# brendan-duncan/unity_webgpu_pathtracer

Measured on AMD Instinct MI355X. Metric: Mrays/s at 1920x1080, 8 spp, higher is better.
Workload: dtype f32; 1 GPU; sponza: Sponza-class atrium (~250k tris, 24 textured Disney materials, 2 rect lights + sky), 1920x1080, 8 spp/pass, depth 4, progressive passes (CurrentSample = 8k); tris=250752, schedule=1, passes_in_flight=12, passes_per_launch_sequence=1

## Files before the change

### unity_webgpu_pathtracer_amd/csrc/pt_device.h

```cpp
#pragma once

#include <hip/hip_runtime.h>
#include <stdint.h>
#include "ptmi_layouts.h"
#include "ptmi_math.h"
#include "ptmi_plugin.h"

#define PT_DEV __device__ __forceinline__

struct v2 { float x, y; };
struct v3 { float x, y, z; };
struct v4 { float x, y, z, w; };

PT_DEV v3 mk3(float a) { return {a, a, a}; }
PT_DEV v3 mk3(float a, float b, float c) { return {a, b, c}; }
PT_DEV v3 operator+(v3 a, v3 b) { return {a.x + b.x, a.y + b.y, a.z + b.z}; }
PT_DEV v3 operator-(v3 a, v3 b) { return {a.x - b.x, a.y - b.y, a.z - b.z}; }
PT_DEV v3 operator-(v3 a) { return {-a.x, -a.y, -a.z}; }
PT_DEV v3 operator*(v3 a, v3 b) { return {a.x * b.x, a.y * b.y, a.z * b.z}; }
PT_DEV v3 operator*(v3 a, float s) { return {a.x * s, a.y * s, a.z * s}; }
PT_DEV v3 operator*(float s, v3 a) { return {s * a.x, s * a.y, s * a.z}; }
PT_DEV v3 operator/(v3 a, float s) { return {a.x / s, a.y / s, a.z / s}; }
PT_DEV v3 operator-(float s, v3 a) { return {s - a.x, s - a.y, s - a.z}; }
PT_DEV v4 operator+(v4 a, v4 b) { return {a.x + b.x, a.y + b.y, a.z + b.z, a.w + b.w}; }
// ... 1232 lines not shown
    v3 Li = light.emission * falloff;
    out.dir = lsDirection;
    out.valid = 1u;
    float pdf = 0.0f;
    v3 f = eval_brdf_onb(mat, -rayDir, lsDirection, onb_of_normal(hit.normal, hit.ffnormal, ffOnb), pdf, sh);
    float lightPdf = 1.0f;
    if (lsPdf > 0.0f) lightPdf = lsPdf;
    out.contribution = Li * f / lightPdf;
}

PT_DEV v4 mul44(const float* m, v4 v)
{
    v4 r;
    r.x = m[0] * v.x + m[4] * v.y + m[8] * v.z + m[12] * v.w;
    r.y = m[1] * v.x + m[5] * v.y + m[9] * v.z + m[13] * v.w;
    r.z = m[2] * v.x + m[6] * v.y + m[10] * v.z + m[14] * v.w;
    r.w = m[3] * v.x + m[7] * v.y + m[11] * v.z + m[15] * v.w;
    return r;
}

PT_DEV void concentric_sample_disk(float u1, float u2, float& dx, float& dy)
{
    float sx = 2.0f * u1 - 1.0f;
    float sy = 2.0f * u2 - 1.0f;
    if (sx == 0.0f && sy == 0.0f) { dx = 0.0f; dy = 0.0f; return; }
    float r, theta;
    if (sx >= -sy) {
        if (sx > sy) { r = sx; theta = sy > 0.0f ? sy / r : 8.0f + sy / r; }
        else { r = sy; theta = 2.0f - sx / r; }
    } else {
        if (sx <= sy) { r = -sx; theta = 4.0f - sy / r; }
        else { r = -sy; theta = 6.0f + sx / r; }
    }
    theta *= PT_PI / 4.0f;
    dx = r * pt_cos(theta);
    dy = r * pt_sin(theta);
}

PT_DEV void generate_camera_ray(const PTFrameParams& P, uint32_t pixelX, uint32_t pixelY, uint32_t& rng, v3& origin, v3& direction)
{
    float g0 = rnd(rng);
    float g1 = rnd(rng);
    float gr = pt_sqrt(-2.0f * pt_log(pt_max(1e-38f, g0)));
    float gtheta = 2.0f * PT_PI * g1;
    float gx = gr * pt_cos(gtheta), gy = gr * pt_sin(gtheta);
    float pcx = (float)pixelX + (0.5f + PT_AA_SIGMA * gx);
    float pcy = (float)pixelY + (0.5f + PT_AA_SIGMA * gy);

    v4 o4 = mul44(P.CamToWorld, v4{0.0f, 0.0f, 0.0f, 1.0f});
    origin = mk3(o4.x, o4.y, o4.z);
    float uvx = pcx / (float)P.OutputWidth * 2.0f - 1.0f;
    float uvy = pcy / (float)P.OutputHeight * 2.0f - 1.0f;
    v4 d4 = mul44(P.CamInvProj, v4{uvx, uvy, 0.0f, 1.0f});
    v4 w4 = mul44(P.CamToWorld, v4{d4.x, d4.y, d4.z, 0.0f});
    direction = normalize3(mk3(w4.x, w4.y, w4.z));
    if (P.Aperture > 0.0f && P.FocalLength > 0.0f) {
        float sampleLensU = rnd(rng);
        float sampleLensV = rnd(rng);
        float lensU, lensV;
        concentric_sample_disk(sampleLensU, sampleLensV, lensU, lensV);
        float lensRadius = P.Aperture * 0.5f;
        lensU *= lensRadius;
        lensV *= lensRadius;
        float ft = P.FocalLength;
        v3 focalPoint = origin + direction * ft;
        v4 l4 = mul44(P.CamToWorld, v4{lensU, lensV, 0.0f, 1.0f});
        origin = mk3(l4.x, l4.y, l4.z);
        direction = normalize3(focalPoint - origin);
    }
}

enum : uint32_t { PS_TRACE = 0u, PS_ENDING = 1u, PS_DONE = 2u };

struct PathRegs {
    v3 ro, rd;
    v3 radiance, throughput, color;
    float scatterPdf, maxRoughness;
    uint32_t rng, depth, state, sampleIdx;
    NeeRay env, light;
    v3 neeOrigin, pendThroughput;
    bool hasPending, green;
};

PT_DEV void path_start_sample(const PTFrameParams& P, uint32_t pixelX, uint32_t pixelY, PathRegs& r, Counters& cn)
{
    cn.paths++;
    r.radiance = mk3(0.0f);
    r.throughput = mk3(1.0f);
    r.depth = 0u;
    r.scatterPdf = 0.0f;
    r.maxRoughness = 0.0f;
    generate_camera_ray(P, pixelX, pixelY, r.rng, r.ro, r.rd);
    r.state = PS_TRACE;
}

PT_DEV void path_init(const PTFrameParams& P, uint32_t seedRoot, uint32_t currentSample, uint32_t pixelX, uint32_t pixelY, uint32_t pixelIndex,
                      PathRegs& r, Counters& cn)
{
    r.rng = pixelIndex * (currentSample + 1u) + seedRoot;
    r.sampleIdx = 0u;
    r.color = mk3(0.0f);
    r.env.valid = 0u; r.light.valid = 0u;
    r.env.dir = mk3(0.0f); r.light.dir = mk3(0.0f);
    r.env.contribution = mk3(0.0f); r.light.contribution = mk3(0.0f);
    r.neeOrigin = mk3(0.0f); r.pendThroughput = mk3(0.0f);
    r.hasPending = false; r.green = false;
    path_start_sample(P, pixelX, pixelY, r, cn);
}

struct NoNeeSink { PT_DEV void operator()(PathRegs&) const {} };
struct CameraSample {
    PT_DEV void operator()(const PTFrameParams& P, uint32_t pixelX, uint32_t pixelY, PathRegs& r, Counters& cn) const { path_start_sample(P, pixelX, pixelY, r, cn); }
};

PT_DEV void path_apply_pending(PathRegs& r, bool occEnv, bool occLight)
{
    if (r.hasPending) {
        v3 Ld = mk3(0.0f);
        if (r.env.valid == 1u && !occEnv) Ld = Ld + r.env.contribution;
        if (r.light.valid == 1u && !occLight) Ld = Ld + r.light.contribution;
        r.radiance = r.radiance + Ld * r.pendThroughput;
        if (r.green) r.radiance = mk3(0.0f, 1.0f, 0.0f);
        r.hasPending = false;
        r.green = false;
    }
}

template <bool STATS, class NeeSink = NoNeeSink>
PT_DEV void path_shade_hit(const DScene& S, const PTFrameParams& P, PathRegs& r, const HitRecord& rec, Counters& cn, NeeSink neeSink = NeeSink())
{
    {
        const uint32_t maxRayBounces = P.MaxRayBounces > 1u ? P.MaxRayBounces : 1u;
        SurfHit hit;
        hit.distance = PT_FAR_PLANE;
        hit.isLight = 0u;
        hit.triIndex = 0u;
        hit.materialIndex = 0;
        hit.position = mk3(0.0f); hit.normal = mk3(0.0f); hit.ffnormal = mk3(0.0f);
        hit.uv = {0.0f, 0.0f};
        if (rec.h.t < PT_FAR_PLANE) {
            if (S.hasTlas) fetch_hit_attributes_tlas(S, r.rd, rec, hit);
            else fetch_hit_attributes<STATS>(S, r.ro, r.rd, rec.h, hit, cn);
        }
        intersect_lights<STATS>(S, r.ro, r.rd, hit, cn);

        if (!(hit.distance < PT_FAR_PLANE)) {
            v4 sky = sample_sky_radiance(S, P, r.rd, r.depth);
            float misWeight = 1.0f;
            if (r.depth > 0u) misWeight = power_heuristic(r.scatterPdf, sky.w);
            if (misWeight > 0.0f) r.radiance = r.radiance + misWeight * mk3(sky.x, sky.y, sky.z) * r.throughput;
            r.state = PS_ENDING;
        } else if (S.hasLights && hit.isLight) {
            DLight light = load_light(S, (int)hit.triIndex);
            if (STATS) cn.lightFetches++;
            r.radiance = r.radiance + light.emission * r.throughput;
            r.state = PS_ENDING;
        } else {
            Material material = get_material<STATS>(S, hit.materialIndex, r.rd, hit, cn);
            r.maxRoughness = pt_max(r.maxRoughness, material.roughness);
            material.roughness = r.maxRoughness;
            r.radiance = r.radiance + material.emission * r.throughput;
            if (r.depth >= maxRayBounces) {
                r.state = PS_ENDING;
            } else {
                v3 scatterL;
                const float alphaRnd = rnd(r.rng);
                const bool skip = (material.alphaMode == (float)PT_ALPHA_MODE_MASK && material.opacity < material.alphaCutoff) ||
                                  (material.alphaMode == (float)PT_ALPHA_MODE_BLEND && alphaRnd > material.opacity);
                bool advance = true;
                if (skip) {
                    scatterL = r.rd;
                } else {
                    r.neeOrigin = nee_scatter_pos(hit);
                    BsdfShared sh;
                    tint_colors(material, material.eta, sh.F0, sh.Csheen, sh.Cspec0);
                    const Onb ffOnb = make_onb(hit.ffnormal);
                    nee_prepare_environment(S, P, r.rd, hit, material, r.rng, r.env, sh, ffOnb);
                    nee_prepare_light<STATS>(S, r.rd, hit, material, r.neeOrigin, r.rng, r.light, cn, sh, ffOnb);
                    r.pendThroughput = r.throughput;
                    r.hasPending = true;
                    neeSink(r);
                    float pdf;
                    v3 f = sample_brdf(material, -r.rd, ffOnb, scatterL, pdf, r.rng, sh);
                    r.scatterPdf = pdf;
                    if (pt_isnan(f.x) || pt_isnan(f.y) || pt_isnan(f.z)) {
                        r.green = true;
                        r.state = PS_ENDING;
                        advance = false;
                    } else if (pdf > 0.0f) {
                        r.throughput = r.throughput * (f / pdf);
                    } else {
                        r.state = PS_ENDING;
                        advance = false;
                    }
                    if (advance) r.depth++;
                }
                if (advance) {
                    r.rd = scatterL;
                    r.ro = hit.position + r.rd * PT_EPSILON;
                    if (P.UseRussianRoulette) {
                        float rrPcont = pt_min(pt_max(r.throughput.x, pt_max(r.throughput.y, r.throughput.z)) + 0.001f, 0.95f);
                        if (rnd(r.rng) >= rrPcont) r.state = PS_ENDING;
                        else r.throughput = r.throughput / rrPcont;
                    }
                }
            }
        }
    }
}

template <bool INLINE_RESOLVE, class Source = CameraSample>
PT_DEV void path_end_sample(const PTFrameParams& P, PathRegs& r, uint32_t pixelX, uint32_t pixelY, uint32_t pixelIndex,
                            const float4* __restrict__ accumulated, float4* __restrict__ output, Counters& cn, Source source = Source())
{
    if (r.state == PS_ENDING && !r.hasPending) {
        if (P.UseFireflyFilter) {
            float lum = luminance3(r.radiance);
            if (lum > P.MaxFireflyLuminance) r.radiance = r.radiance * (P.MaxFireflyLuminance / lum);
        }
        r.color = r.color + r.radiance;
        r.sampleIdx++;
        const uint32_t numSamples = P.SamplesPerPass > 1 ? (uint32_t)P.SamplesPerPass : 1u;
        if (r.sampleIdx < numSamples) {
            source(P, pixelX, pixelY, r, cn);
        } else if (!INLINE_RESOLVE) {
            r.state = PS_DONE;
        } else {
            const float fSamples = (float)numSamples;
            float4 o4;
            if (P.CurrentSample > 0u) {
                float4 a = accumulated[pixelIndex];
                cn.pixelsRead++;
                float cs = (float)P.CurrentSample;
                v3 acc = (r.color + mk3(a.x, a.y, a.z) * cs) / (cs + fSamples);
                o4 = make_float4(acc.x, acc.y, acc.z, 1.0f);
            } else {
                v3 acc = r.color / fSamples;
                o4 = make_float4(acc.x, acc.y, acc.z, 1.0f);
            }
            output[pixelIndex] = o4;
            cn.pixelsWritten++;
            r.state = PS_DONE;
        }
    }
}

template <bool STATS, bool INLINE_RESOLVE = true, class NeeSink = NoNeeSink, class Source = CameraSample>
PT_DEV void path_step(const DScene& S, const PTFrameParams& P, PathRegs& r, const HitRecord& rec, bool occEnv, bool occLight,
                      uint32_t pixelX, uint32_t pixelY, uint32_t pixelIndex,
                      const float4* __restrict__ accumulated, float4* __restrict__ output, Counters& cn, NeeSink neeSink = NeeSink(),
                      Source source = Source())
{
    path_apply_pending(r, occEnv, occLight);
    if (r.state == PS_TRACE) path_shade_hit<STATS, NeeSink>(S, P, r, rec, cn, neeSink);
    path_end_sample<INLINE_RESOLVE, Source>(P, r, pixelX, pixelY, pixelIndex, accumulated, output, cn, source);
}

PT_DEV uint32_t wave_sum_u32(uint32_t v)
{
#pragma unroll
    for (int off = 32; off > 0; off >>= 1) v += __shfl_xor(v, off, 64);
    return v;
}
PT_DEV uint32_t wave_max_u32(uint32_t v)
{
#pragma unroll
    for (int off = 32; off > 0; off >>= 1) { uint32_t o = __shfl_xor(v, off, 64); v = o > v ? o : v; }
    return v;
}
#define PT_NUM_COUNTERS 16
PT_DEV void counters_to_array(const Counters& cn, uint32_t* vals)
{
    vals[0] = cn.paths; vals[1] = cn.closestRays; vals[2] = cn.shadowRays; vals[3] = cn.nodeVisits; vals[4] = cn.triTests;
    vals[5] = cn.attrFetches; vals[6] = cn.materialFetches; vals[7] = cn.lightFetches; vals[8] = cn.texelFetches;
    vals[9] = cn.texDescFetches; vals[10] = cn.pixelsWritten; vals[11] = cn.pixelsRead; vals[12] = cn.maxStack; vals[13] = cn.overflows;
    vals[14] = cn.tlasNodeVisits; vals[15] = cn.instanceVisits;
}

template <bool STATS, class ST>
PT_DEV bool ray_step(const DScene& S, RayState& r, ST& st, Counters& cn)
{
    return cwbvh_iteration<STATS, false>(S, r, BlasOffsets{}, st, cn);
}

template <bool STATS>
PT_DEV bool ray_tri_one(const DScene& S, RayState& r, Counters& cn)
{
    const uint32_t triangleIndex = 31u - (uint32_t)__clz((int)r.tg.y);
    intersect_triangle<false>(S.tris, r.tg.x + triangleIndex * 3u, 0u, r.o, r.d, r.hit);
    if (STATS) cn.triTests++;
    r.tg.y -= 1u << triangleIndex;
    if (r.anyHit && r.hit.t < PT_FAR_PLANE) {
        if (STATS && r.overflow) cn.overflows++;
        return true;
    }
    return false;
}

template <bool STATS, class ST>
PT_DEV bool ray_node_one(const DScene& S, RayState& r, ST& st, Counters& cn)
{
    if (r.ng.y <= 0x00FFFFFFu) {
        if (r.sp > 0u) { --r.sp; r.ng = stack_pop(st, r.sp); }
        else {
            if (STATS && r.overflow) cn.overflows++;
            return true;
        }
    }
    if (r.ng.y > 0x00FFFFFFu) {
        cwbvh_visit_node<STATS>(S.nodes, 0u, r.o, r.invDir, r.octinv4, r.hit.t, r.ng, r.tg, r.sp, r.overflow, st, cn);
    } else {
        r.tg = r.ng;
        r.ng = make_uint2(0u, 0u);
    }
    return false;
}
```

### unity_webgpu_pathtracer_amd/csrc/pt_wavefront.hip

```cpp
#include "pt_device.h"
#include "pt_launch.h"
#include <type_traits>

namespace {

#define PT_WF_CHUNK 64u
#define PT_WF_SHARDS 8u

PT_DEV uint32_t pack_flags(const PathRegs& r)
{
    return (r.state & 3u) | ((r.hasPending ? 1u : 0u) << 2) | ((r.env.valid & 3u) << 3) | ((r.light.valid & 1u) << 5) |
           ((r.green ? 1u : 0u) << 6) | ((r.sampleIdx & 0xFFFu) << 7) | ((r.depth & 0x1FFFu) << 19);
}
PT_DEV uint32_t fl_state(uint32_t f) { return f & 3u; }
PT_DEV bool fl_pending(uint32_t f) { return (f >> 2) & 1u; }
PT_DEV uint32_t fl_env(uint32_t f) { return (f >> 3) & 3u; }
PT_DEV uint32_t fl_light(uint32_t f) { return (f >> 5) & 1u; }

PT_DEV float4 f4(v3 v, float w) { return make_float4(v.x, v.y, v.z, w); }
PT_DEV v3 xyz(float4 v) { return mk3(v.x, v.y, v.z); }

PT_DEV float4* f4_array(const PTWfBuffers& B, uint32_t k) { return B.f4base + (size_t)k * B.f4stride; }
PT_DEV void fetch_ray(const PTWfBuffers& B, uint32_t slot, uint32_t kind, v3& o, v3& d)
{
    const float4* rec = f4_array(B, 2u * kind) + 2u * (size_t)slot;
    o = xyz(rec[0]);
    d = xyz(rec[1]);
}

PT_DEV void store_path(const PTWfBuffers& B, uint32_t slot, const PathRegs& r, bool writeNee)
{
    B.flags[slot] = pack_flags(r);
    B.rng[slot] = r.rng;
    B.ray[0][2u * slot] = f4(r.ro, r.scatterPdf);
    B.ray[0][2u * slot + 1u] = f4(r.rd, r.maxRoughness);
    B.rad[slot] = f4(r.radiance, 0.0f);
    B.thr[slot] = f4(r.throughput, 0.0f);
    B.color[slot] = f4(r.color, 0.0f);
    if (writeNee) {
        B.ray[1][2u * slot] = f4(r.neeOrigin, 0.0f);
        B.ray[1][2u * slot + 1u] = f4(r.env.dir, 0.0f);
        B.ray[2][2u * slot] = f4(r.neeOrigin, 0.0f);
        B.ray[2][2u * slot + 1u] = f4(r.light.dir, 0.0f);
        B.envC[slot] = f4(r.env.contribution, 0.0f);
        B.lightC[slot] = f4(r.light.contribution, 0.0f);
        B.pthr[slot] = f4(r.pendThroughput, 0.0f);
    }
}

template <bool STATS>
PT_DEV void flush_counters(const Counters& cn, unsigned long long* rows, uint32_t row, uint32_t lane)
{
    uint32_t vals[PT_NUM_COUNTERS];
    counters_to_array(cn, vals);
    unsigned long long* p = rows + (size_t)row * 16u;
#pragma unroll
    for (int i = 0; i < PT_NUM_COUNTERS; ++i) {
        if (!STATS && (i >= 3 && i <= 9)) continue;
        if (!STATS && i >= 12) continue;
        if (i == 12) {
            uint32_t m = wave_max_u32(vals[i]);
            if (lane == 0 && m > p[i]) p[i] = m;
        } else {
            uint32_t s = wave_sum_u32(vals[i]);
            if (lane == 0 && s) p[i] += s;
        }
    }
}

PT_DEV uint32_t pixel_slot_of(const PTWfBuffers& B, uint32_t slot, uint32_t& pass)
{
    pass = 0u;
    if (slot >= B.slotsPerPass) { pass = slot / B.slotsPerPass; slot -= pass * B.slotsPerPass; }
    return slot;
}

PT_DEV bool wf_pixel(const PTTileMap& tm, const PTWfBuffers& B, uint32_t slot, uint32_t wgSlot, uint32_t& px, uint32_t& py, uint32_t& pass, uint32_t& base)
{
    base = 0u;
    return pt_slot_to_pixel(tm, pixel_slot_of(B, slot, pass), px, py);
}
PT_DEV bool wf_pixel(const PTListMap& lm, const PTWfBuffers& B, uint32_t slot, uint32_t wgSlot, uint32_t& px, uint32_t& py, uint32_t& pass, uint32_t& base)
{
    pass = wgSlot / B.slotsPerPass;
    const uint2 entry = lm.table[(wgSlot - pass * B.slotsPerPass) >> 8];
    base = entry.y;
    return pt_list_slot_to_pixel(lm.frameBlocksX, lm.coverW, lm.coverH, entry.x, slot & 255u, px, py);
}
template <class MAP> constexpr bool kListMap = std::is_same<MAP, PTListMap>::value;

PT_DEV bool wf_pixel(const PTRayMap& rm, const PTWfBuffers& B, uint32_t slot, uint32_t wgSlot, uint32_t& px, uint32_t& py, uint32_t& pass, uint32_t& base)
{
    px = 0u; py = 0u; pass = 0u; base = 0u;
    return slot < rm.count;
}
template <class MAP> constexpr bool kRayMap = std::is_same<MAP, PTRayMap>::value;
struct RaySample {
    const PTRadianceRay* rays; uint32_t slot;
    PT_DEV void operator()(const PTFrameParams&, uint32_t, uint32_t, PathRegs& r, Counters& cn) const { start(r, cn); }
    PT_DEV void start(PathRegs& r, Counters& cn) const
    {
        const float4* e = (const float4*)(rays + slot);
        const float4 a = e[0], b = e[1];
        cn.paths++;
        r.radiance = mk3(0.0f);
        r.throughput = mk3(1.0f);
        r.depth = 0u;
        r.scatterPdf = 0.0f;
        r.maxRoughness = 0.0f;
        r.ro = mk3(a.x, a.y, a.z);
        r.rd = mk3(a.w, b.x, b.y);
        r.state = PS_TRACE;
    }
};
PT_DEV void ray_path_init(const PTRayMap& rm, uint32_t slot, PathRegs& r, Counters& cn)
{
    r.rng = rm.rays[slot].rng;
    r.sampleIdx = 0u;
    r.color = mk3(0.0f);
    r.env.valid = 0u; r.light.valid = 0u;
    r.env.dir = mk3(0.0f); r.light.dir = mk3(0.0f);
    r.env.contribution = mk3(0.0f); r.light.contribution = mk3(0.0f);
    r.neeOrigin = mk3(0.0f); r.pendThroughput = mk3(0.0f);
    r.hasPending = false; r.green = false;
    RaySample{rm.rays, slot}.start(r, cn);
}

template <class MAP = PTTileMap>
__global__ __launch_bounds__(256) void pt_wf_init(PTFrameParams P, PTBatch batch, MAP tm, PTWfBuffers B)
{
    const uint32_t slot = blockIdx.x * 256u + threadIdx.x;
    if (blockIdx.x == 0u && threadIdx.x < PT_WF_SHARDS) B.chunkHeads[threadIdx.x * 32u] = 0u;
    if (slot >= B.numSlots) return;
    uint32_t px, py, pass, base;
    Counters cn = {};
    if (!wf_pixel(tm, B, slot, blockIdx.x * 256u, px, py, pass, base)) B.flags[slot] = PS_DONE;
    else {
        PathRegs r;
        if constexpr (kRayMap<MAP>) ray_path_init(tm, slot, r, cn);
        else {
            uint32_t seedRoot, currentSample;
            pt_batch_pick(batch, pass, seedRoot, currentSample);
            if (kListMap<MAP>) currentSample = base + pass * (P.SamplesPerPass > 1 ? (uint32_t)P.SamplesPerPass : 1u);
            path_init(P, seedRoot, currentSample, px, py, py * P.OutputWidth + px, r, cn);
        }
        store_path(B, slot, r, false);
    }
    flush_counters<false>(cn, B.statRows, blockIdx.x * 4u + (threadIdx.x >> 6), threadIdx.x & 63u);
}

#ifndef PT_WF_TRACE_MIN_WAVES
#define PT_WF_TRACE_MIN_WAVES 8
#endif

template <bool STATS, bool TLAS>
__global__ __launch_bounds__(256, 4) void pt_wf_trace(DScene S, PTWfBuffers B, uint32_t iteration)
{
    __shared__ uint2 s_stack[PT_LDS_STACK][256];
    const uint32_t nb = B.numSlots >> 8;
    const uint32_t vb = blockIdx.x;
    const uint32_t kind = vb / nb;
    const uint32_t slot = (vb % nb) * 256u + threadIdx.x;
    const uint32_t f = B.flags[slot];
    bool valid;
    if (kind == 0u) valid = fl_state(f) == PS_TRACE;
    else if (kind == 1u) valid = fl_pending(f) && fl_env(f) != 0u;
    else valid = fl_pending(f) && fl_light(f) != 0u;
    Counters cn = {};
    if (valid) {
        v3 o, d;
        fetch_ray(B, slot, kind, o, d);
        TravStack st;
        st.lds = PT_LDS_U2(&s_stack[0][threadIdx.x]);
        st.stride = 256u;
        HitRecord h;
        h.h.t = PT_FAR_PLANE; h.h.u = 0.0f; h.h.v = 0.0f; h.h.triIndex = 0u;
        h.pos = mk3(0.0f); h.inst = 0u;
        bool occluded;
        if (TLAS) occluded = traverse_tlas<STATS>(S, o, d, kind != 0u, h, st, cn);
        else { traverse_cwbvh<STATS>(S, o, d, kind != 0u, h.h, st, cn); occluded = h.h.t < PT_FAR_PLANE; }
        if (kind == 0u) {
            B.hit[slot] = make_float4(h.h.t, h.h.u, h.h.v, pt_asfloat(h.h.triIndex));
            if (TLAS) B.hit2[slot] = make_float4(h.pos.x, h.pos.y, h.pos.z, pt_asfloat(h.inst));
            cn.closestRays++;
        } else { B.occl[(size_t)(kind - 1u) * B.numSlots + slot] = occluded ? 1 : 0; cn.shadowRays++; }
    }
    flush_counters<STATS>(cn, B.statRows, (B.numSlots >> 6) + vb * 4u + (threadIdx.x >> 6), threadIdx.x & 63u);
}

#ifndef PT_WF_RANGE
#define PT_WF_RANGE 128u
#endif
#define PT_WF_STAT_ROW_SETS 4u
static_assert(PT_WF_RANGE >= 64u && (PT_WF_RANGE & (PT_WF_RANGE - 1u)) == 0u && PT_WF_STAT_ROW_SETS >= 3u,
              "one counter row per trace wave: the main trace launch uses rows numSlots/64 + wave, the tail launch rows 2 x numSlots/64 + wave");
#ifndef PT_WF_REFILL
#define PT_WF_REFILL 16u
#endif
#ifndef PT_WF_TRI_PARK
#define PT_WF_TRI_PARK 4u
#endif

typedef volatile __attribute__((address_space(3))) uint32_t* pt_lds_u32;
typedef volatile __attribute__((address_space(3))) uint16_t* pt_lds_u16;
PT_DEV uint32_t rank_below(unsigned long long m)
{
    return __builtin_amdgcn_mbcnt_hi((uint32_t)(m >> 32), __builtin_amdgcn_mbcnt_lo((uint32_t)m, 0u));
}
// ... 520 lines not shown
#define PT_WF_SHADE_MIN_WAVES 3
#endif

PT_DEV void load_path(const PTWfBuffers& B, uint32_t slot, uint32_t f, PathRegs& r)
{
    r.state = fl_state(f);
    r.hasPending = fl_pending(f);
    r.env.valid = fl_env(f);
    r.light.valid = fl_light(f);
    r.green = (f >> 6) & 1u;
    r.sampleIdx = (f >> 7) & 0xFFFu;
    r.depth = f >> 19;
    r.rng = B.rng[slot];
    float4 q;
    q = B.ray[0][2u * slot]; r.ro = xyz(q); r.scatterPdf = q.w;
    q = B.ray[0][2u * slot + 1u]; r.rd = xyz(q); r.maxRoughness = q.w;
    r.radiance = xyz(B.rad[slot]);
    r.throughput = xyz(B.thr[slot]);
    r.color = xyz(B.color[slot]);
    r.env.dir = mk3(0.0f); r.light.dir = mk3(0.0f); r.neeOrigin = mk3(0.0f);
    r.env.contribution = mk3(0.0f); r.light.contribution = mk3(0.0f); r.pendThroughput = mk3(0.0f);
    if (r.hasPending) {
        r.env.contribution = xyz(B.envC[slot]);
        r.light.contribution = xyz(B.lightC[slot]);
        r.pendThroughput = xyz(B.pthr[slot]);
    }
}

template <bool STATS, bool PIXSUM = false, class MAP = PTTileMap>
PT_DEV bool shade_slot(const DScene& S, const PTFrameParams& P, const MAP& tm, const PTWfBuffers& B, uint32_t slot, uint32_t pixelSlot,
                       uint32_t f, Counters& cn, uint32_t wgSlot = 0u)
{
    uint32_t px, py, pass, base;
    wf_pixel(tm, B, pixelSlot, wgSlot, px, py, pass, base);
    uint32_t rng = B.rng[slot];
    float4 qro = B.ray[0][2u * slot], qrd = B.ray[0][2u * slot + 1u], qrad = B.rad[slot], qthr = B.thr[slot], qcol = B.color[slot];
    float4 qenvC = B.envC[slot], qlightC = B.lightC[slot], qpthr = B.pthr[slot], qhit = B.hit[slot];
    uint32_t o0 = B.occl[slot], o1 = B.occl[(size_t)B.numSlots + slot];
    float4 qhit2 = make_float4(0.0f, 0.0f, 0.0f, 0.0f);
    if (S.hasTlas) qhit2 = B.hit2[slot];
    asm volatile("" : "+v"(rng), "+v"(qro.x), "+v"(qrd.x), "+v"(qrad.x), "+v"(qthr.x), "+v"(qcol.x), "+v"(qenvC.x), "+v"(qlightC.x), "+v"(qpthr.x),
                      "+v"(qhit.x), "+v"(o0), "+v"(o1), "+v"(qhit2.x));
    PathRegs r;
    r.state = fl_state(f);
    r.hasPending = fl_pending(f);
    r.env.valid = fl_env(f);
    r.light.valid = fl_light(f);
    r.green = (f >> 6) & 1u;
    r.sampleIdx = (f >> 7) & 0xFFFu;
    r.depth = f >> 19;
    r.rng = rng;
    r.ro = xyz(qro); r.scatterPdf = qro.w;
    r.rd = xyz(qrd); r.maxRoughness = qrd.w;
    r.radiance = xyz(qrad);
    r.throughput = xyz(qthr);
    r.color = xyz(qcol);
    r.env.dir = mk3(0.0f); r.light.dir = mk3(0.0f); r.neeOrigin = mk3(0.0f);
    r.env.contribution = r.hasPending ? xyz(qenvC) : mk3(0.0f);
    r.light.contribution = r.hasPending ? xyz(qlightC) : mk3(0.0f);
    r.pendThroughput = r.hasPending ? xyz(qpthr) : mk3(0.0f);
    const bool occEnv = r.hasPending && o0 != 0u, occLight = r.hasPending && o1 != 0u;
    HitRecord ch;
    ch.h.t = PT_FAR_PLANE; ch.h.u = 0.0f; ch.h.v = 0.0f; ch.h.triIndex = 0u;
    ch.pos = mk3(0.0f); ch.inst = 0u;
    if (r.state == PS_TRACE) {
        ch.h.t = qhit.x; ch.h.u = qhit.y; ch.h.v = qhit.z; ch.h.triIndex = pt_asuint(qhit.w);
        if (S.hasTlas) { ch.pos = xyz(qhit2); ch.inst = pt_asuint(qhit2.w); }
    }
    struct Sink {
        const PTWfBuffers& B; uint32_t slot;
        PT_DEV void operator()(PathRegs& q) const {
            uint32_t s2 = slot;
            asm volatile("" : "+v"(s2));
            B.ray[1][2u * s2] = f4(q.neeOrigin, 0.0f);
            B.ray[1][2u * s2 + 1u] = f4(q.env.dir, 0.0f);
            B.ray[2][2u * s2] = f4(q.neeOrigin, 0.0f);
            B.ray[2][2u * s2 + 1u] = f4(q.light.dir, 0.0f);
            B.envC[s2] = f4(q.env.contribution, 0.0f);
            B.lightC[s2] = f4(q.light.contribution, 0.0f);
            B.pthr[s2] = f4(q.pendThroughput, 0.0f);
        }
    };
    if constexpr (kRayMap<MAP>)
        path_step<STATS, false, Sink, RaySample>(S, P, r, ch, occEnv, occLight, 0u, 0u, 0u, nullptr, nullptr, cn, Sink{B, slot}, RaySample{tm.rays, pixelSlot});
    else
        path_step<STATS, false, Sink>(S, P, r, ch, occEnv, occLight, px, py, py * P.OutputWidth + px, nullptr, nullptr, cn, Sink{B, slot});
    uint32_t storeSlot = slot;
    asm volatile("" : "+v"(storeSlot));
    store_path(B, storeSlot, r, false);
    if (PIXSUM && r.state == PS_DONE) {
        uint32_t ps = pixelSlot;
        asm volatile("" : "+v"(ps));
        B.pixsum[ps] = f4(r.color, 0.0f);
    }
    return r.state != PS_DONE;
}

#ifndef PT_WF_SHADE_BLOCK
#define PT_WF_SHADE_BLOCK 64u
#endif
template <bool STATS, class MAP = PTTileMap>
__global__ __launch_bounds__(PT_WF_SHADE_BLOCK, PT_WF_SHADE_MIN_WAVES) void pt_wf_shade(DScene S, PTFrameParams P, MAP tm, PTWfBuffers B,
                                                                         uint32_t iteration)
{
    const uint32_t vb = blockIdx.x;
    const uint32_t slot = vb * PT_WF_SHADE_BLOCK + threadIdx.x;
    if (vb == 0u && threadIdx.x < PT_WF_SHARDS) B.chunkHeads[threadIdx.x * 32u] = 0u;
    const uint32_t f = B.flags[slot];
    Counters cn = {};
    if (fl_state(f) != PS_DONE) shade_slot<STATS, false, MAP>(S, P, tm, B, slot, slot, f, cn, vb * PT_WF_SHADE_BLOCK);
    flush_counters<STATS>(cn, B.statRows, vb * (PT_WF_SHADE_BLOCK / 64u) + (threadIdx.x >> 6), threadIdx.x & 63u);
}

#ifndef PT_WF_FUSED_WAVES
#define PT_WF_FUSED_WAVES 4
#endif

#define PT_WF_NO_PIXEL 0xFFFFFFFFu

template <bool STATS>
PT_DEV void counters_to_lds(const Counters& cn, pt_lds_u32 tot, uint32_t lane)
{
    uint32_t vals[PT_NUM_COUNTERS];
    counters_to_array(cn, vals);
#pragma unroll
    for (int i = 0; i < PT_NUM_COUNTERS; ++i) {
        if (!STATS && (i >= 3 && i <= 9)) continue;
        if (!STATS && i >= 12) continue;
        if (i == 12) {
            const uint32_t m = wave_max_u32(vals[i]);
            if (lane == 0u && m > tot[i]) tot[i] = m;
        } else {
            const uint32_t v = wave_sum_u32(vals[i]);
            if (lane == 0u && v) tot[i] += v;
        }
    }
}

template <bool STATS>
__global__ __launch_bounds__(64, PT_WF_FUSED_WAVES) void pt_wf_fused(DScene S, PTFrameParams P, PTBatch batch, PTTileMap tm, PTWfBuffers B)
{
    constexpr uint32_t K = PT_WF_FUSED_GROUPS;
    constexpr uint32_t kSusp = PT_WF_SUSPEND ? PT_WF_SUSPEND : 1u;
    static_assert((K & (K - 1u)) == 0u && K >= 1u && K <= 16u, "context groups per wave: a power of two");
    __shared__ uint2 s_stack[PT_WF_LDS_STACK][64];
    __shared__ uint32_t s_xchg[64];
    __shared__ uint32_t s_pix[K][64];
    __shared__ uint32_t s_pend[2][K][2];
    __shared__ uint4 s_susp[kSusp][PT_WF_SUSP_ROWS];
    __shared__ uint32_t s_cnt[PT_NUM_COUNTERS];
    __shared__ uint32_t s_gw;
    const uint32_t lane = threadIdx.x;
    const uint32_t ctxBase = blockIdx.x * (K * 64u);
    pt_lds_u32 xchg = (pt_lds_u32)&s_xchg[0];
    pt_lds_u32 pix = (pt_lds_u32)&s_pix[0][0];
    pt_lds_u32 cnt = (pt_lds_u32)&s_cnt[0];
#pragma unroll
    for (uint32_t k = 0; k < K; ++k) {
        s_pix[k][lane] = PT_WF_NO_PIXEL;
        B.flags[ctxBase + k * 64u + lane] = PS_DONE;
    }
    if (lane < PT_NUM_COUNTERS) s_cnt[lane] = 0u;
    if (lane < 4u * K) (&s_pend[0][0][0])[lane] = 0u;
    if (lane == 0u) s_gw = blockIdx.x;
    __builtin_amdgcn_wave_barrier();
    uint32_t nSusp = 0u, pb = 0u;
    bool more = true;

    while (true) {
// ... 104 lines not shown
                        have = false;
                    }
                    nSusp = (uint32_t)__popcll(act);
                    break;
                }
            }
            pb = pn;
            counters_to_lds<STATS>(cn, cnt, lane);
        }
        __builtin_amdgcn_fence(__ATOMIC_RELEASE, "workgroup");
        __builtin_amdgcn_fence(__ATOMIC_ACQUIRE, "workgroup");
        __builtin_amdgcn_wave_barrier();

#pragma unroll 1
        for (uint32_t k = 0; k < K; ++k) {
            const uint32_t ctx = ctxBase + k * 64u + lane;
            const uint32_t mine = pix[k * 64u + lane];
            const uint32_t pw = s_pend[pb][k][lane >> 5];
            const bool parked = (pw >> (lane & 31u)) & 1u;
            Counters cn = {};
            if (mine != PT_WF_NO_PIXEL && !parked) {
                const uint32_t f = B.flags[ctx];
                if (!shade_slot<STATS, true>(S, P, tm, B, ctx, mine, f, cn)) pix[k * 64u + lane] = PT_WF_NO_PIXEL;
            }
            counters_to_lds<STATS>(cn, cnt, lane);
        }
        __builtin_amdgcn_fence(__ATOMIC_RELEASE, "workgroup");
        __builtin_amdgcn_fence(__ATOMIC_ACQUIRE, "workgroup");
        __builtin_amdgcn_wave_barrier();
    }
    __builtin_amdgcn_wave_barrier();
    if (lane < PT_NUM_COUNTERS) {
        unsigned long long* p = B.statRows + (size_t)blockIdx.x * 16u + lane;
        const unsigned long long v = cnt[lane];
        if (lane == 12u) { if (v > *p) *p = v; } else if (v) *p += v;
    }
}

template <bool STATS, bool TLAS, class MAP = PTTileMap>
__global__ __launch_bounds__(256, 2) void pt_wf_cleanup(DScene S, PTFrameParams P, MAP tm, PTWfBuffers B)
{
    __shared__ uint2 s_stack[PT_LDS_STACK][256];
    Counters cn = {};
    for (uint32_t blk = blockIdx.x; blk < (B.numSlots >> 8); blk += gridDim.x) {
    const uint32_t slot = blk * 256u + threadIdx.x;
    const uint32_t f = B.flags[slot];
    if (__any(fl_state(f) != PS_DONE)) {
        if (fl_state(f) != PS_DONE) {
            uint32_t px, py, pass, base;
            wf_pixel(tm, B, slot, blk * 256u, px, py, pass, base);
            PathRegs r;
            load_path(B, slot, f, r);
            if (r.hasPending) {
                r.neeOrigin = xyz(B.ray[1][2u * slot]);
                r.env.dir = xyz(B.ray[1][2u * slot + 1u]);
                r.light.dir = xyz(B.ray[2][2u * slot + 1u]);
            }
            TravStack st;
            st.lds = PT_LDS_U2(&s_stack[0][threadIdx.x]);
            st.stride = 256u;
            while (r.state != PS_DONE) {
                HitRecord ch;
                ch.h.t = PT_FAR_PLANE; ch.h.u = 0.0f; ch.h.v = 0.0f; ch.h.triIndex = 0u;
                ch.pos = mk3(0.0f); ch.inst = 0u;
                bool occEnv = false, occLight = false;
                if (r.hasPending && r.env.valid != 0u) {
                    HitRecord h = ch;
                    if (TLAS) occEnv = traverse_tlas<STATS>(S, r.neeOrigin, r.env.dir, true, h, st, cn);
                    else { traverse_cwbvh<STATS>(S, r.neeOrigin, r.env.dir, true, h.h, st, cn); occEnv = h.h.t < PT_FAR_PLANE; }
                    cn.shadowRays++;
                }
                if (r.hasPending && r.light.valid != 0u) {
                    HitRecord h = ch;
                    if (TLAS) occLight = traverse_tlas<STATS>(S, r.neeOrigin, r.light.dir, true, h, st, cn);
                    else { traverse_cwbvh<STATS>(S, r.neeOrigin, r.light.dir, true, h.h, st, cn); occLight = h.h.t < PT_FAR_PLANE; }
                    cn.shadowRays++;
                }
                if (r.state == PS_TRACE) {
                    if (TLAS) traverse_tlas<STATS>(S, r.ro, r.rd, false, ch, st, cn);
                    else traverse_cwbvh<STATS>(S, r.ro, r.rd, false, ch.h, st, cn);
                    cn.closestRays++;
                }
                if constexpr (kRayMap<MAP>)
                    path_step<STATS, false, NoNeeSink, RaySample>(S, P, r, ch, occEnv, occLight, 0u, 0u, 0u, nullptr, nullptr, cn, NoNeeSink(), RaySample{tm.rays, slot});
                else
                    path_step<STATS, false>(S, P, r, ch, occEnv, occLight, px, py, py * P.OutputWidth + px, nullptr, nullptr, cn);
            }
            B.flags[slot] = pack_flags(r);
            B.color[slot] = f4(r.color, 0.0f);
            if constexpr (kRayMap<MAP>) B.rng[slot] = r.rng;
        }
    }
    }
    flush_counters<STATS>(cn, B.statRows, blockIdx.x * 4u + (threadIdx.x >> 6), threadIdx.x & 63u);
}

template <class MAP = PTTileMap>
__global__ __launch_bounds__(256) void pt_wf_resolve(PTFrameParams P, PTBatch batch, MAP tm, PTWfBuffers B, const float4* __restrict__ sums,
                                                     const float4* __restrict__ accumulated, float4* __restrict__ output)
{
    const uint32_t slot = blockIdx.x * 256u + threadIdx.x;
    uint32_t px, py, pass, base;
    Counters cn = {};
    if (slot < B.slotsPerPass && wf_pixel(tm, B, slot, blockIdx.x * 256u, px, py, pass, base)) {
        const uint32_t pixelIndex = py * P.OutputWidth + px;
        const uint32_t numSamples = P.SamplesPerPass > 1 ? (uint32_t)P.SamplesPerPass : 1u;
        const float fSamples = (float)numSamples;
        v3 acc = mk3(0.0f);
        for (uint32_t j = 0; j < batch.count; ++j) {
            uint32_t seedRoot, currentSample;
            pt_batch_pick(batch, j, seedRoot, currentSample);
            if (kListMap<MAP>) currentSample = base + j * numSamples;
            const v3 color = xyz(sums[(size_t)j * B.slotsPerPass + slot]);
            if (currentSample > 0u) {
                if (j == 0u) {
                    const float4 a = accumulated[pixelIndex];
                    acc = mk3(a.x, a.y, a.z);
                }
                cn.pixelsRead++;
                const float cs = (float)currentSample;
                acc = (color + acc * cs) / (cs + fSamples);
            } else {
                acc = color / fSamples;
            }
            cn.pixelsWritten++;
        }
        output[pixelIndex] = make_float4(acc.x, acc.y, acc.z, 1.0f);
    }
    flush_counters<false>(cn, B.statRows, blockIdx.x * 4u + (threadIdx.x >> 6), threadIdx.x & 63u);
}

__global__ __launch_bounds__(256) void pt_wf_resolve_rays(PTFrameParams P, PTRayMap rm, PTWfBuffers B, PTRadiance* __restrict__ out)
{
    const uint32_t slot = blockIdx.x * 256u + threadIdx.x;
    if (slot >= rm.count) return;
    const uint32_t numSamples = P.SamplesPerPass > 1 ? (uint32_t)P.SamplesPerPass : 1u;
    const float fSamples = (float)numSamples;
    const v3 acc = xyz(B.color[slot]) / fSamples;
    ((float4*)out)[slot] = make_float4(acc.x, acc.y, acc.z, pt_asfloat(B.rng[slot]));
}

__global__ __launch_bounds__(256) void pt_wf_fold_rows(unsigned long long* rows, uint32_t numRows, unsigned long long* gstats)
{
    unsigned long long acc[PT_NUM_COUNTERS] = {};
    for (uint32_t r = blockIdx.x * 256u + threadIdx.x; r < numRows; r += gridDim.x * 256u) {
        unsigned long long* p = rows + (size_t)r * 16u;
#pragma unroll
        for (int i = 0; i < PT_NUM_COUNTERS; ++i) {
            unsigned long long v = p[i];
            if (i == 12) acc[i] = v > acc[i] ? v : acc[i]; else acc[i] += v;
            p[i] = 0ull;
        }
    }
    const uint32_t lane = threadIdx.x & 63u;
#pragma unroll
    for (int i = 0; i < PT_NUM_COUNTERS; ++i) {
        unsigned long long v = acc[i];
        for (int off = 32; off > 0; off >>= 1) {
            unsigned long long o = __shfl_xor(v, off, 64);
            if (i == 12) v = o > v ? o : v; else v += o;
        }
        if (lane == 0 && v) { if (i == 12) atomicMax(&gstats[i], v); else atomicAdd(&gstats[i], v); }
    }
}

size_t pt_wf_arena_layout(char* base, uint32_t numSlots, uint32_t residentWaves, bool needTlas, uint32_t maxIterations, PTWfBuffers& B)
{
    const size_t n = numSlots;
    const uint32_t numRows = PT_WF_STAT_ROW_SETS * (numSlots >> 6);
// ... 195 lines not shown
```

Before: 5515 Mrays/s.

## Overlap next sample's camera ray with pending shadow rays of the ending sample

When a path is ending but still has pending NEE shadow rays, the wavefront shade step now starts the next sample's camera ray at once instead of waiting an extra iteration. The pending shadow result is folded into the previous sample's color on the next step, before the new hit is shaded. This removes one wavefront iteration per sample boundary where a lane would trace only shadow rays. The cost is extra state logic in path_step, and accumulation could break if the overlapped flag is misdetected.

New measurement: 5766 Mrays/s (median of 6 runs). +4.6%, better.

```diff
diff --git a/unity_webgpu_pathtracer_amd/csrc/pt_device.h b/unity_webgpu_pathtracer_amd/csrc/pt_device.h
--- a/unity_webgpu_pathtracer_amd/csrc/pt_device.h
+++ b/unity_webgpu_pathtracer_amd/csrc/pt_device.h
@@ -1338,17 +1338,26 @@
     bool hasPending, green;
 };
 
-PT_DEV void path_start_sample(const PTFrameParams& P, uint32_t pixelX, uint32_t pixelY, PathRegs& r, Counters& cn)
-{
-    cn.paths++;
+PT_DEV void path_reset_sample(PathRegs& r)
+{
     r.radiance = mk3(0.0f);
     r.throughput = mk3(1.0f);
     r.depth = 0u;
+}
+PT_DEV void path_start_ray(const PTFrameParams& P, uint32_t pixelX, uint32_t pixelY, PathRegs& r, Counters& cn)
+{
+    cn.paths++;
     r.scatterPdf = 0.0f;
     r.maxRoughness = 0.0f;
     generate_camera_ray(P, pixelX, pixelY, r.rng, r.ro, r.rd);
     r.state = PS_TRACE;
 }
+PT_DEV void path_start_sample(const PTFrameParams& P, uint32_t pixelX, uint32_t pixelY, PathRegs& r, Counters& cn)
+{
+    path_reset_sample(r);
+    path_start_ray(P, pixelX, pixelY, r, cn);
+}
+PT_DEV bool path_overlapped(const PathRegs& r) { return r.state == PS_TRACE && r.hasPending && r.depth == 0u; }
 
 PT_DEV void path_init(const PTFrameParams& P, uint32_t seedRoot, uint32_t currentSample, uint32_t pixelX, uint32_t pixelY, uint32_t pixelIndex,
                       PathRegs& r, Counters& cn)
@@ -1366,7 +1375,7 @@
 
 struct NoNeeSink { PT_DEV void operator()(PathRegs&) const {} };
 struct CameraSample {
-    PT_DEV void operator()(const PTFrameParams& P, uint32_t pixelX, uint32_t pixelY, PathRegs& r, Counters& cn) const { path_start_sample(P, pixelX, pixelY, r, cn); }
+    PT_DEV void operator()(const PTFrameParams& P, uint32_t pixelX, uint32_t pixelY, PathRegs& r, Counters& cn) const { path_start_ray(P, pixelX, pixelY, r, cn); }
 };
 
 PT_DEV void path_apply_pending(PathRegs& r, bool occEnv, bool occLight)
@@ -1465,20 +1474,27 @@
     }
 }
 
-template <bool INLINE_RESOLVE, class Source = CameraSample>
+PT_DEV void path_fold_sample(const PTFrameParams& P, PathRegs& r)
+{
+    if (P.UseFireflyFilter) {
+        float lum = luminance3(r.radiance);
+        if (lum > P.MaxFireflyLuminance) r.radiance = r.radiance * (P.MaxFireflyLuminance / lum);
+    }
+    r.color = r.color + r.radiance;
+    r.sampleIdx++;
+}
+
+template <bool INLINE_RESOLVE, class Source = CameraSample, bool OVERLAP = false>
 PT_DEV void path_end_sample(const PTFrameParams& P, PathRegs& r, uint32_t pixelX, uint32_t pixelY, uint32_t pixelIndex,
                             const float4* __restrict__ accumulated, float4* __restrict__ output, Counters& cn, Source source = Source())
 {
+    bool startRay = false;
     if (r.state == PS_ENDING && !r.hasPending) {
-        if (P.UseFireflyFilter) {
-            float lum = luminance3(r.radiance);
-            if (lum > P.MaxFireflyLuminance) r.radiance = r.radiance * (P.MaxFireflyLuminance / lum);
-        }
-        r.color = r.color + r.radiance;
-        r.sampleIdx++;
+        path_fold_sample(P, r);
         const uint32_t numSamples = P.SamplesPerPass > 1 ? (uint32_t)P.SamplesPerPass : 1u;
         if (r.sampleIdx < numSamples) {
-            source(P, pixelX, pixelY, r, cn);
+            path_reset_sample(r);
+            startRay = true;
         } else if (!INLINE_RESOLVE) {
             r.state = PS_DONE;
         } else {
@@ -1498,18 +1514,27 @@
             cn.pixelsWritten++;
             r.state = PS_DONE;
         }
-    }
-}
-
-template <bool STATS, bool INLINE_RESOLVE = true, class NeeSink = NoNeeSink, class Source = CameraSample>
+    } else if (OVERLAP && r.state == PS_ENDING && r.sampleIdx + 1u < (P.SamplesPerPass > 1 ? (uint32_t)P.SamplesPerPass : 1u)) {
+        r.depth = 0u;
+        startRay = true;
+    }
+    if (startRay) source(P, pixelX, pixelY, r, cn);
+}
+
+template <bool STATS, bool INLINE_RESOLVE = true, class NeeSink = NoNeeSink, class Source = CameraSample, bool OVERLAP = false>
 PT_DEV void path_step(const DScene& S, const PTFrameParams& P, PathRegs& r, const HitRecord& rec, bool occEnv, bool occLight,
                       uint32_t pixelX, uint32_t pixelY, uint32_t pixelIndex,
                       const float4* __restrict__ accumulated, float4* __restrict__ output, Counters& cn, NeeSink neeSink = NeeSink(),
                       Source source = Source())
 {
+    const bool deferred = OVERLAP && path_overlapped(r);
     path_apply_pending(r, occEnv, occLight);
+    if (deferred) {
+        path_fold_sample(P, r);
+        path_reset_sample(r);
+    }
     if (r.state == PS_TRACE) path_shade_hit<STATS, NeeSink>(S, P, r, rec, cn, neeSink);
-    path_end_sample<INLINE_RESOLVE, Source>(P, r, pixelX, pixelY, pixelIndex, accumulated, output, cn, source);
+    path_end_sample<INLINE_RESOLVE, Source, OVERLAP>(P, r, pixelX, pixelY, pixelIndex, accumulated, output, cn, source);
 }
 
 PT_DEV uint32_t wave_sum_u32(uint32_t v)
diff --git a/unity_webgpu_pathtracer_amd/csrc/pt_wavefront.hip b/unity_webgpu_pathtracer_amd/csrc/pt_wavefront.hip
--- a/unity_webgpu_pathtracer_amd/csrc/pt_wavefront.hip
+++ b/unity_webgpu_pathtracer_amd/csrc/pt_wavefront.hip
@@ -97,15 +97,12 @@
 template <class MAP> constexpr bool kRayMap = std::is_same<MAP, PTRayMap>::value;
 struct RaySample {
     const PTRadianceRay* rays; uint32_t slot;
-    PT_DEV void operator()(const PTFrameParams&, uint32_t, uint32_t, PathRegs& r, Counters& cn) const { start(r, cn); }
-    PT_DEV void start(PathRegs& r, Counters& cn) const
+    PT_DEV void operator()(const PTFrameParams&, uint32_t, uint32_t, PathRegs& r, Counters& cn) const { start_ray(r, cn); }
+    PT_DEV void start_ray(PathRegs& r, Counters& cn) const
     {
         const float4* e = (const float4*)(rays + slot);
         const float4 a = e[0], b = e[1];
         cn.paths++;
-        r.radiance = mk3(0.0f);
-        r.throughput = mk3(1.0f);
-        r.depth = 0u;
         r.scatterPdf = 0.0f;
         r.maxRoughness = 0.0f;
         r.ro = mk3(a.x, a.y, a.z);
@@ -123,7 +120,8 @@
     r.env.contribution = mk3(0.0f); r.light.contribution = mk3(0.0f);
     r.neeOrigin = mk3(0.0f); r.pendThroughput = mk3(0.0f);
     r.hasPending = false; r.green = false;
-    RaySample{rm.rays, slot}.start(r, cn);
+    path_reset_sample(r);
+    RaySample{rm.rays, slot}.start_ray(r, cn);
 }
 
 template <class MAP = PTTileMap>
@@ -810,9 +808,9 @@
         }
     };
     if constexpr (kRayMap<MAP>)
-        path_step<STATS, false, Sink, RaySample>(S, P, r, ch, occEnv, occLight, 0u, 0u, 0u, nullptr, nullptr, cn, Sink{B, slot}, RaySample{tm.rays, pixelSlot});
+        path_step<STATS, false, Sink, RaySample, true>(S, P, r, ch, occEnv, occLight, 0u, 0u, 0u, nullptr, nullptr, cn, Sink{B, slot}, RaySample{tm.rays, pixelSlot});
     else
-        path_step<STATS, false, Sink>(S, P, r, ch, occEnv, occLight, px, py, py * P.OutputWidth + px, nullptr, nullptr, cn, Sink{B, slot});
+        path_step<STATS, false, Sink, CameraSample, true>(S, P, r, ch, occEnv, occLight, px, py, py * P.OutputWidth + px, nullptr, nullptr, cn, Sink{B, slot});
     uint32_t storeSlot = slot;
     asm volatile("" : "+v"(storeSlot));
     store_path(B, storeSlot, r, false);
@@ -1083,9 +1081,9 @@
                     cn.closestRays++;
                 }
                 if constexpr (kRayMap<MAP>)
-                    path_step<STATS, false, NoNeeSink, RaySample>(S, P, r, ch, occEnv, occLight, 0u, 0u, 0u, nullptr, nullptr, cn, NoNeeSink(), RaySample{tm.rays, slot});
+                    path_step<STATS, false, NoNeeSink, RaySample, true>(S, P, r, ch, occEnv, occLight, 0u, 0u, 0u, nullptr, nullptr, cn, NoNeeSink(), RaySample{tm.rays, slot});
                 else
-                    path_step<STATS, false>(S, P, r, ch, occEnv, occLight, px, py, py * P.OutputWidth + px, nullptr, nullptr, cn);
+                    path_step<STATS, false, NoNeeSink, CameraSample, true>(S, P, r, ch, occEnv, occLight, px, py, py * P.OutputWidth + px, nullptr, nullptr, cn);
             }
             B.flags[slot] = pack_flags(r);
             B.color[slot] = f4(r.color, 0.0f);
```
